# Yujia-Yan/Transkun

Hardware: AMD Instinct MI355X
Metric: semi-CRF logProb+backward steps/sec at T=1024, NBatch=352 (higher is better)
Workload: dtype f32; 1 GPU; NeuralSemiCRFInterval(score, noise).logProb(intervals) fwd+bwd through the public API (Python interval lists packed inside the timed region), T=1024, NBatch=352 per GPU, fp32, exact-hash randn-like scores resident in HBM; T=1024, NBatch=352, impl=0, parallelism=chains sharded, 1 rank(s) seen by the process group, no data-path collective

## Files before the change

transkun_amd/csrc/persist.hip:

```cpp
#include <atomic>
#include <stdlib.h>
#include "common.h"
#include "pathscore.h"

#ifndef SEMICRF_PANEL_PROBES
#define SEMICRF_PANEL_PROBES 0
#endif

#ifndef SEMICRF_PROBE_TASKS
#define SEMICRF_PROBE_TASKS 0
#endif
#ifndef SEMICRF_PROBE_HIST
#define SEMICRF_PROBE_HIST 0
#endif

#ifndef SEMICRF_CT_DBG
#define SEMICRF_CT_DBG -1
#endif

namespace semicrf {

constexpr int PB = 16;
#ifndef SEMICRF_RING
#define SEMICRF_RING 4
#endif
constexpr int RING = SEMICRF_RING;
#ifndef SEMICRF_NNEAR
#define SEMICRF_NNEAR 0
#endif
constexpr int NNEAR = SEMICRF_NNEAR;
#ifndef SEMICRF_BANDX
#define SEMICRF_BANDX 1
#endif
#ifndef SEMICRF_BANDX_MAXB
#define SEMICRF_BANDX_MAXB 192
#endif
#ifndef SEMICRF_BAND_LOAD_AUX
#define SEMICRF_BAND_LOAD_AUX 16
#endif
#ifndef SEMICRF_BANDX_WGSTRIDE
#define SEMICRF_BANDX_WGSTRIDE 3
#endif
#ifndef SEMICRF_BANDX_WAVES
#define SEMICRF_BANDX_WAVES 1
#endif
#ifndef SEMICRF_BANDX_K0
#define SEMICRF_BANDX_K0 8
#endif
constexpr int NBT = RING + NNEAR;
constexpr int FAR0 = RING + NNEAR;
constexpr int RS = 4;
constexpr int GS = RS;
constexpr int GP = 32;
#ifndef SEMICRF_TPT
#define SEMICRF_TPT 12
#endif
constexpr int TPT = SEMICRF_TPT;
#ifndef SEMICRF_LEADT
#define SEMICRF_LEADT 4
#endif
constexpr int LEADT = SEMICRF_LEADT;
__host__ __device__ inline int nfull_of(int q) { return q + 1 - LEADT >= 0 ? (q + 1 - LEADT) / TPT : 0; }
__host__ __device__ inline int nparts_of(int q) { return nfull_of(q) + 1; }
__host__ __device__ inline void part_tiles(int q, int part, int& m0, int& m1)
{
    m0 = part * TPT;
    m1 = part < nfull_of(q) ? m0 + TPT : q + 1;
}
#ifndef SEMICRF_NT
#define SEMICRF_NT 640
#endif
constexpr int NT = SEMICRF_NT;
constexpr int MAX_CHUNKS = 16;
constexpr float LOG2E = 1.4426950408889634f;
constexpr float LN2 = 0.6931471805599453f;
constexpr int SPIN_LIMIT = 1 << 20;
constexpr int SPIN_LIMIT_LDS = 1 << 24;
constexpr float RESC_LIFT = 96.0f, RESC_HI = 108.0f, RESC_EARLY = 56.0f;
constexpr unsigned CTRL_INIT = 0xffffffffu;
constexpr unsigned U_EMPTY = 0xffffffffu;

constexpr size_t CTRL_WORDS = 256;
constexpr int CTRL_EXIT = 64;
constexpr int CTRL_COPYQ = 192;
constexpr int CTRL_PATHQ = 160;
constexpr int CTRL_GEN = 96;

typedef unsigned long long u64;
typedef unsigned v4u __attribute__((ext_vector_type(4)));
typedef unsigned v4u_a4 __attribute__((ext_vector_type(4), aligned(4)));
template <int V>
struct IC { static constexpr int value = V; };

#define DBGF(P) (SEMICRF_CT_DBG >= 0 ? (unsigned)SEMICRF_CT_DBG : (P).dbg)
struct SweepParams {
    const float* score;
    const float* noise;
    int T, B, K;
    int c0, c1;
    int nSpine, nPanelGroups;
    int nTasks;
    int taskBase;
    int panelWaves;
    int hybridPanelWaves;
    int hybridStart;
    int zeroWaves;
    unsigned tag;
    int selfclean;
    unsigned expect_gen;
    unsigned dbg;
    unsigned* ctrl;
    u64* ts;
    unsigned* ug;
    unsigned* ug_other;
    int gradLazyShort;
    int bandWaves;
    u64* farg;
    float* u_out;
    float* last_out;
    int* code;
    const float* vfwd;
    const float* logZ;
    const float* gout;
    int gstride;
    float gscale;
    float* dScore;
    float* dNoise;
    const int* pathPairs;
    const int* pathOffsets;
    int pathK;
    int pathSpine;
    float* pathOut;
    u64* pathg;
    float noiseAdd;
    float* band;
    unsigned* bandFlags;
    int bandSpines;
    int bandGroups;
    int bandK0;
    int copyWaves;
    int cellNT;
    int gradNT;
    int nfarw;
};

__device__ __forceinline__ float fexp2(float x) { return __builtin_amdgcn_exp2f(x); }
__device__ __forceinline__ float flog2(float x) { return __builtin_amdgcn_logf(x); }

__device__ __forceinline__ u64 make_granule(unsigned tag, float v)
{
    return ((u64)tag << 32) | (u64)__float_as_uint(v);
}
__device__ __forceinline__ u64 make_granule_key(unsigned tag, float v, int key)
{
    return ((u64)(((tag & 0xffffu) << 16) | ((unsigned)key & 0xffffu)) << 32) | (u64)__float_as_uint(v);
}
__device__ __forceinline__ void store_granule(u64* p, u64 g)
{
    __hip_atomic_store(p, g, __ATOMIC_RELAXED, __HIP_MEMORY_SCOPE_AGENT);
}
__device__ __forceinline__ u64 load_granule(const u64* p)
{
    return __hip_atomic_load(p, __ATOMIC_RELAXED, __HIP_MEMORY_SCOPE_AGENT);
}

template <int DIR>
__device__ __forceinline__ int frame_of(int p, int T) { return DIR == 0 ? p : T - 1 - p; }

template <int DIR>
__device__ __forceinline__ size_t cell_index(int pi, int pj, int T)
{
    return DIR == 0 ? (size_t)pi * T + pj : (size_t)(T - 1 - pj) * T + (T - 1 - pi);
}
template <int DIR>
__device__ __forceinline__ int gap_of(int p, int T) { return DIR == 0 ? p - 1 : T - 1 - p; }

__device__ __forceinline__ void acc_push1(float& M, float& S, float t)
{
    const float d = t - M;
    const float e = fexp2(-fabsf(d));
    S = d > 0.0f ? fmaf(S, e, 1.0f) : S + e;
    M = fmaxf(M, t);
}
__device__ __forceinline__ void acc_merge(float& M, float& S, float M2, float S2)
{
    if (S2 == 0.0f) return;
    if (M2 > M) {
        S = S * fexp2(M - M2) + S2;
        M = M2;
    } else {
        S += S2 * fexp2(M2 - M);
    }
}
template <int DIR>
__device__ __forceinline__ void max_push_seq(float& best, int& key, float t, int k)
{
    const bool take = DIR == 0 ? t > best : t >= best;
    best = take ? t : best;
    key = take ? k : key;
}
__device__ __forceinline__ float softplus2(float x)
{
    const float x2 = x * LOG2E;
    return x > 20.0f ? x2 : flog2(1.0f + fexp2(x2));
}

__device__ unsigned g_dev_status = 0;
__shared__ int s_abort;

__device__ unsigned* g_host_abort = nullptr;

__device__ __forceinline__ void set_error(unsigned* ctrl, unsigned code)
{
    __hip_atomic_store(ctrl + 1, code, __ATOMIC_RELAXED, __HIP_MEMORY_SCOPE_AGENT);
    __hip_atomic_store(&g_dev_status, code, __ATOMIC_RELAXED, __HIP_MEMORY_SCOPE_AGENT);
    unsigned* const h = g_host_abort;
    if (h) __hip_atomic_store(h, code, __ATOMIC_RELAXED, __HIP_MEMORY_SCOPE_SYSTEM);
}

__device__ __forceinline__ bool spin_abort(unsigned* ctrl, int& spins, int limit, unsigned code)
{
    ++spins;
    if (spins > limit) { set_error(ctrl, code); s_abort = 1; return true; }
    if ((spins & 255) == 0 &&
        __hip_atomic_load(ctrl + 1, __ATOMIC_RELAXED, __HIP_MEMORY_SCOPE_AGENT) != CTRL_INIT) { s_abort = 1; return true; }
    return false;
}

#ifndef SEMICRF_NLOADER
#define SEMICRF_NLOADER 1
#endif
constexpr int NLOADER = SEMICRF_NLOADER;
#ifndef SEMICRF_NRBUF
#define SEMICRF_NRBUF 4
#endif
constexpr int NRBUF = SEMICRF_NRBUF;
constexpr int TILE_BYTES = PB * PB * RS * 4;
constexpr int NCONST = 3;
constexpr int LDS_TILES = 0;
constexpr int LDS_CONST = LDS_TILES + NRBUF * RING * TILE_BYTES;
constexpr int LDS_FAR = LDS_CONST + NRBUF * NCONST * 256;
constexpr int NFAR = 8;
constexpr int NPOS = 128;
static_assert(NFAR >= RING && NPOS >= RING * PB, "ring geometry");
constexpr int LDS_RING = LDS_FAR + NFAR * 64 * 16;
#ifndef SEMICRF_STAGGER
#define SEMICRF_STAGGER 32
#endif
#ifndef SEMICRF_GRAD_LAZY
#define SEMICRF_GRAD_LAZY 127
#endif
#ifndef SEMICRF_GRAD_HSTART
#define SEMICRF_GRAD_HSTART 12
#endif
#ifndef SEMICRF_LOADER_PACE
#define SEMICRF_LOADER_PACE 0
#endif
#ifndef SEMICRF_LOADER_AUX
#define SEMICRF_LOADER_AUX 0
#endif
#ifndef SEMICRF_SPH
#define SEMICRF_SPH 1
#endif
#ifndef SEMICRF_FAR_EARLY
#define SEMICRF_FAR_EARLY 0
#endif
#ifndef SEMICRF_FAR_PRIO
#define SEMICRF_FAR_PRIO 0
#endif
#ifndef SEMICRF_NFARW
#define SEMICRF_NFARW 2
#endif
constexpr int NFARW = SEMICRF_NFARW;
constexpr int NNSLOT = 8;
constexpr int NEAR_SLOT_BYTES = NNEAR * TILE_BYTES + 256;
constexpr int LDS_NEAR = LDS_RING + NPOS * RS * 8;
constexpr int LDS_CTL = LDS_NEAR + (NNEAR > 0 ? NNSLOT * NEAR_SLOT_BYTES : 0);
static_assert(NPOS >= (FAR0 + 1) * PB && NNSLOT >= FAR0 + 1 && NRBUF + RING + NNSLOT + NFARW <= 64 && NNSLOT % NFARW == 0, "near geometry");
constexpr int LDS_DUMMY = LDS_CTL + 256;
constexpr int LDS_SPINE_BYTES = LDS_DUMMY + (64 * 2 + PB * 8) * 4;

typedef __attribute__((address_space(3))) void lds_void_t;
typedef __attribute__((address_space(1))) const void gbl_void_t;

struct SpineBlk { float v[PB]; };

__device__ __forceinline__ int spine_row(int lane) { return lane & 15; }
__device__ __forceinline__ int spine_chain(int lane) { return lane >> 4; }

template <int N>
__device__ __forceinline__ void wait_vmcnt() { asm volatile("s_waitcnt vmcnt(%0)" ::"n"(N)); }

__device__ __forceinline__ int lds_flag_load(const int* p) { return __hip_atomic_load(p, __ATOMIC_RELAXED, __HIP_MEMORY_SCOPE_WORKGROUP); }
__device__ __forceinline__ void lds_flag_store(int* p, int v) { __hip_atomic_store(p, v, __ATOMIC_RELAXED, __HIP_MEMORY_SCOPE_WORKGROUP); }
__device__ __forceinline__ unsigned lds_addr(const void* p)
{
    return (unsigned)(uintptr_t)(__attribute__((address_space(3))) const void*)p;
}
__device__ __forceinline__ int lds_flag_load_asm(const int* p)
{
    int v;
    asm volatile("ds_read_b32 %0, %1\n\ts_waitcnt lgkmcnt(0)" : "=v"(v) : "v"(lds_addr(p)) : "memory");
    return v;
}
__device__ __forceinline__ void lds_flag_store_asm(int* p, int v)
{
    asm volatile("ds_write_b32 %0, %1" ::"v"(lds_addr(p)), "v"(v) : "memory");
}
__device__ __forceinline__ u64 lds_load64(const void* p)
{
    return __hip_atomic_load((const u64*)p, __ATOMIC_RELAXED, __HIP_MEMORY_SCOPE_WORKGROUP);
}
__device__ __forceinline__ void lds_store64(void* p, float value, int seq)
{
    __hip_atomic_store((u64*)p, ((u64)(unsigned)seq << 32) | (u64)__float_as_uint(value), __ATOMIC_RELAXED, __HIP_MEMORY_SCOPE_WORKGROUP);
}
typedef float f32x4_t __attribute__((ext_vector_type(4)));
__device__ __forceinline__ void lds_store128(void* p, float4 v)
{
    const f32x4_t w = {v.x, v.y, v.z, v.w};
    asm volatile("ds_write_b128 %0, %1" ::"v"(lds_addr(p)), "v"(w) : "memory");
}
__device__ __forceinline__ float4 lds_load128(const void* p)
{
    f32x4_t w;
    asm volatile("ds_read_b128 %0, %1\n\ts_waitcnt lgkmcnt(0)" : "=v"(w) : "v"(lds_addr(p)) : "memory");
    return make_float4(w.x, w.y, w.z, w.w);
}

template <int DIR, bool GRAD>
__device__ __forceinline__ void loader_role(const SweepParams& P, int sg, char* lds, int lid)
{
    const int T = P.T, B = P.B, K = P.K;
    unsigned* const ctrl = P.ctrl;
    const size_t Bs = (size_t)B;
    const float* const score = P.score;
    const float* const noise = P.noise;
    const float* const vfwd = P.vfwd;
    const int lane = threadIdx.x & 63;
    const int cbase = P.c0 + sg * GS;
    const size_t last4 = (size_t)T * T * Bs - 4;
    const int tu = lane >> 4, tr = lane & 15;
    const int cr = spine_row(lane), cch = spine_chain(lane);
    const int cc = cbase + cch < P.c1 ? cbase + cch : cbase;
    int* const ready = (int*)(lds + LDS_CTL);
    int* const cons = ready + NRBUF;
    int* const nready = cons + RING;
    const int* const fcons = nready + NNSLOT;
    constexpr int NL = RING * 4 + 2 + (GRAD ? 1 : 0) + NNEAR * 4 + ((GRAD && NNEAR > 0) ? 1 : 0);
    constexpr int LDEPTH = 3 * NL <= 63 ? 3 : 2;
    static_assert(2 * NL <= 63, "loader pipeline");

    const bool useband = SEMICRF_BANDX && P.band != nullptr;
    const float* const bandp = useband ? P.band + (size_t)(cbase / GS) * NBT * (TILE_BYTES / 4) + lane * 4 : nullptr;
    const size_t band_kr = (size_t)P.bandSpines * NBT * (TILE_BYTES / 4);
    typedef unsigned v16u __attribute__((ext_vector_type(16)));
    const int bKpad = K + 2;
    const unsigned* const bflags = useband ? P.bandFlags + (size_t)(cbase / GP) * bKpad * 8 : nullptr;
    const unsigned btag = P.tag;
    int ready_upto = -1;
    auto band_ready = [&](int kr) -> bool {
        const uintptr_t fa = (uintptr_t)(bflags + (size_t)kr * 8);
        const u64 fp = (u64)(unsigned)__builtin_amdgcn_readfirstlane((int)(unsigned)fa) |
                       ((u64)(unsigned)__builtin_amdgcn_readfirstlane((int)(unsigned)(fa >> 32)) << 32);
        v16u f;
        asm volatile("s_load_dwordx16 %0, %1, 0x0 glc\n\ts_waitcnt lgkmcnt(0)" : "=&s"(f) : "s"(fp) : "memory");
        const unsigned want0 = ((btag & 0xffffu) << 16) | (unsigned)kr, want1 = want0 + 1u;
        bool ok0 = true, ok1 = true;
#pragma unroll
        for (int i = 0; i < NBT; ++i) { ok0 = ok0 && f[i] == want0; ok1 = ok1 && f[8 + i] == want1; }
        if (ok0) ready_upto = ok1 ? kr + 1 : kr;
        return ok0;
    };
    auto issue = [&](int kr) {
        const int slot = kr % NRBUF;
        const int prow_t = kr * PB + tr < T ? kr * PB + tr : T - 1;
        const bool fromband = useband && kr >= P.bandK0;
        if (fromband) {
            const float* const bk = bandp + (size_t)kr * band_kr;
#pragma unroll
            for (int i = 0; i < RING; ++i)
#pragma unroll
                for (int q = 0; q < 4; ++q)
                    __builtin_amdgcn_global_load_lds((gbl_void_t*)(bk + i * (TILE_BYTES / 4) + q * 256),
                                                     (lds_void_t*)(lds + LDS_TILES + (slot * RING + i) * TILE_BYTES + q * 1024), 16, 0, SEMICRF_BAND_LOAD_AUX);
// ... 754 lines not shown
        const int c = c0 + g * GP + q8 * 4;
        const bool cvalid = c < c1;
        const int cl = cvalid ? c : c0;

        float aM[4][4], aS[4][4];
        int aK[4][4];
#pragma unroll
        for (int rr = 0; rr < 4; ++rr)
#pragma unroll
            for (int i = 0; i < 4; ++i) { aM[rr][i] = SEMICRF_NEG_INF; aS[rr][i] = 0.f; aK[rr][i] = 0x7fffffff; }

        float arow[4][4], gz[4];
        if (GRAD) {
            float lz[4];
#pragma unroll
            for (int i = 0; i < 4; ++i) {
                const bool ok = c + i < c1;
                lz[i] = ok ? logZp[c + i] : 0.f;
                gz[i] = ok ? goutp[(size_t)(c + i) * P.gstride] * P.gscale : 0.f;
            }
#pragma unroll
            for (int rr = 0; rr < 4; ++rr) {
                const int pi = pbase + rr;
#pragma unroll
                for (int i = 0; i < 4; ++i) {
                    const float vv = (c + i < c1 && pi < T) ? vfwd[(size_t)frame_of<DIR>(pi, T) * Bs + c + i] : 0.f;
                    arow[rr][i] = (vv - lz[i]) * LOG2E;
                }
            }
        }
        PanelGeom G;
        geom_of(tk, G);
        char* const stage0 = lds + wslot * (PNS * PSTAGE_BYTES);
        const unsigned rdbase = lds_addr(stage0) + (DIR == 0 ? (unsigned)lane * 16u
                                                             : (unsigned)((slot >> 1) * 1024 + (slot & 1) * 128 + q8 * 16));
        const unsigned grbase = lds_addr(stage0) + 8192u + (unsigned)lane * 16u;
        const bool probe_stream = SEMICRF_PANEL_PROBES && (dbg & 32u);
        const bool probe_nowait = SEMICRF_PANEL_PROBES && (dbg & 4u);
        const bool probe_nou = SEMICRF_PANEL_PROBES && (dbg & 64u);
        const int nst = GRAD ? 2 * (T - pbase < 4 ? T - pbase : 4) : 0;

        bool frontier = false;
#pragma unroll
        for (int i = 0; i < PNS; ++i)
            if (m0 + i < m1) {
                panel_fetch_cells<DIR>(score, G, stage0 + i * PSTAGE_BYTES, m0 + i, T, Bs, cell_nt);
                if (!probe_stream && !probe_nou) panel_fetch_gran<false>(ursrc, stage0 + i * PSTAGE_BYTES, G.gvoff, m0 + i, B);
                issued += 10;
                if (i == 0) mark0 = issued; else if (i == 1) mark1 = issued; else mark2 = issued;
            }

        for (int m = m0, s = 0; m < m1; ++m, s = (s + 1 == PNS ? 0 : s + 1)) {
            char* const stage = stage0 + s * PSTAGE_BYTES;
            const bool tprobe = SEMICRF_PANEL_PROBES && (dbg & 16u) && g == 0 && q4 == 0 && m == q && lane == 0 && k < 64 && T >= 1024;
            if (tprobe) P.ts[1536 + k] = __builtin_amdgcn_s_memrealtime();
            panel_wait_younger(issued - (s == 0 ? mark0 : (s == 1 ? mark1 : mark2)));
            if (tprobe) P.ts[1600 + k] = __builtin_amdgcn_s_memrealtime();
            int npoll = 0;
            if (tr && m == m0) tsp[1] = __builtin_amdgcn_s_memrealtime();
            if (SEMICRF_PROBE_HIST && (dbg & 1024u) && lane == 0) {
                u64* const hb = P.ts + (3 * T) / 2;
                const u64 now = __builtin_amdgcn_s_memrealtime();
                const u64 t0 = __hip_atomic_load(hb + 129 + (__builtin_amdgcn_s_getreg(6164) & 7), __ATOMIC_RELAXED, __HIP_MEMORY_SCOPE_AGENT);
                u64 b = now > t0 ? (now - t0) / 400 : 0;
                if (b > 63) b = 63;
                atomicAdd((unsigned long long*)(hb + 1 + 64 * hist_role + b), 1ull);
            }
            v4u xo[8];
            panel_read_cells<DIR>(rdbase + (unsigned)(s * PSTAGE_BYTES), xo);
            const bool refill = m + PNS < m1;
            if (probe_stream) {
#pragma unroll
                for (int e = 0; e < 8; ++e)
                    aS[0][0] += __uint_as_float(xo[e].x) + __uint_as_float(xo[e].y) + __uint_as_float(xo[e].z) + __uint_as_float(xo[e].w);
            } else {
                v4u g0, g1;
                panel_read_gran(grbase + (unsigned)(s * PSTAGE_BYTES), g0, g1);
                if (!probe_nowait) {
                    const bool v0 = c < c1, v1 = c + 1 < c1, v2 = c + 2 < c1, v3 = c + 3 < c1;
                    int spins = 0;
                    while (true) {
                        const bool ok = (g0.x != U_EMPTY || !v0) && (g0.y != U_EMPTY || !v1) && (g0.z != U_EMPTY || !v2) &&
                                        (g0.w != U_EMPTY || !v3) && (g1.x != U_EMPTY || !v0) && (g1.y != U_EMPTY || !v1) &&
                                        (g1.z != U_EMPTY || !v2) && (g1.w != U_EMPTY || !v3);
                        if (__all(ok)) break;
                        frontier = true;
                        if (m == q) __builtin_amdgcn_s_sleep(2);
                        else if (GRAD) {
                            if (P.gradLazyShort) __builtin_amdgcn_s_sleep(16);
                            else __builtin_amdgcn_s_sleep(SEMICRF_GRAD_LAZY);
                        }
                        else __builtin_amdgcn_s_sleep(16);
                        if (spin_abort(ctrl, spins, SPIN_LIMIT, 5)) break;
                        ++npoll;
                        if (m == q) panel_fetch_gran<true>(ursrc, stage, G.gvoff, m, B);
                        const unsigned pw = __builtin_amdgcn_raw_buffer_load_b32(ursrc, (unsigned)(cl * 4), (unsigned)((m * PB + PB - 1) * B * 4), 16);
                        if (!__all(pw != U_EMPTY || !cvalid)) continue;
                        if (m != q) panel_fetch_gran<true>(ursrc, stage, G.gvoff, m, B);
                        wait_vmcnt<0>();
                        panel_read_gran(grbase + (unsigned)(s * PSTAGE_BYTES), g0, g1);
                    }
                }
                if (frontier && m + 1 < m1) {
                    const int sn = s + 1 == PNS ? 0 : s + 1;
                    panel_fetch_gran<true>(ursrc, stage0 + sn * PSTAGE_BYTES, G.gvoff, m + 1, B);
                    issued += 2;
                    if (sn == 0) mark0 = issued; else if (sn == 1) mark1 = issued; else mark2 = issued;
                }
                if (SEMICRF_PANEL_PROBES && (dbg & 16u) && g == 0 && q4 == 0 && m == q && lane == 0) P.ts[192 + k] = __builtin_amdgcn_s_memrealtime();
                if (c >= c1) { g0.x = 0u; g1.x = 0u; }
                if (c + 1 >= c1) { g0.y = 0u; g1.y = 0u; }
                if (c + 2 >= c1) { g0.z = 0u; g1.z = 0u; }
                if (c + 3 >= c1) { g0.w = 0u; g1.w = 0u; }
                const float uv[2][4] = {{__uint_as_float(g0.x), __uint_as_float(g0.y), __uint_as_float(g0.z), __uint_as_float(g0.w)},
                                        {__uint_as_float(g1.x), __uint_as_float(g1.y), __uint_as_float(g1.z), __uint_as_float(g1.w)}};

                if (MODE == 0) {
                    typedef float v2f __attribute__((ext_vector_type(2)));
                    const v2f l2e = {LOG2E, LOG2E};
                    const v2f u2[2][2] = {{{uv[0][0], uv[0][1]}, {uv[0][2], uv[0][3]}}, {{uv[1][0], uv[1][1]}, {uv[1][2], uv[1][3]}}};
                    const auto gs = __builtin_amdgcn_make_buffer_rsrc((void*)(GRAD ? dScore + panel_tile_off<DIR>(G, m, T, Bs) : nullptr), 0,
                                                                      0x7fffffff, 0x00020000);
#pragma unroll
                    for (int rr = 0; rr < 4; ++rr) {
                        v2f e[2][2];
#pragma unroll
                        for (int h = 0; h < 2; ++h) {
                            const v4u xv = xo[rr * 2 + h];
                            const v2f x2[2] = {{__uint_as_float(xv.x), __uint_as_float(xv.y)}, {__uint_as_float(xv.z), __uint_as_float(xv.w)}};
#pragma unroll
                            for (int j = 0; j < 2; ++j) {
                                const v2f mj = {aM[rr][2 * j], aM[rr][2 * j + 1]};
                                e[h][j] = __builtin_elementwise_fma(x2[j], l2e, u2[h][j] - mj);
                            }
                        }
                        const float emax = fmaxf(fmaxf(fmaxf(e[0][0].x, e[0][0].y), fmaxf(e[0][1].x, e[0][1].y)),
                                                 fmaxf(fmaxf(e[1][0].x, e[1][0].y), fmaxf(e[1][1].x, e[1][1].y)));
                        if (__any(emax > RESC_HI)) {
#pragma unroll
                            for (int i = 0; i < 4; ++i) {
                                const float x0 = __uint_as_float(i == 0 ? xo[rr * 2].x : (i == 1 ? xo[rr * 2].y : (i == 2 ? xo[rr * 2].z : xo[rr * 2].w)));
                                const float x1 = __uint_as_float(i == 0 ? xo[rr * 2 + 1].x : (i == 1 ? xo[rr * 2 + 1].y : (i == 2 ? xo[rr * 2 + 1].z : xo[rr * 2 + 1].w)));
                                const float t0 = fmaf(x0, LOG2E, uv[0][i]), t1 = fmaf(x1, LOG2E, uv[1][i]);
                                acc_lift(aM[rr][i], aS[rr][i], fmaxf(t0, t1));
                                const float e0 = t0 - aM[rr][i], e1 = t1 - aM[rr][i];
                                if (i & 1) { e[0][i >> 1].y = e0; e[1][i >> 1].y = e1; } else { e[0][i >> 1].x = e0; e[1][i >> 1].x = e1; }
                            }
                        }
                        v2f mg[2][2];
#pragma unroll
                        for (int j = 0; j < 2; ++j) {
                            v2f sj = {aS[rr][2 * j], aS[rr][2 * j + 1]};
                            const v2f p0 = {fexp2(e[0][j].x), fexp2(e[0][j].y)};
                            const v2f p1 = {fexp2(e[1][j].x), fexp2(e[1][j].y)};
                            sj = (sj + p0) + p1;
                            aS[rr][2 * j] = sj.x; aS[rr][2 * j + 1] = sj.y;
                            if (GRAD) {
                                const v2f mj = {aM[rr][2 * j], aM[rr][2 * j + 1]};
                                const v2f aj = {arow[rr][2 * j], arow[rr][2 * j + 1]};
                                const v2f fa = mj + aj;
                                const v2f gzj = {gz[2 * j], gz[2 * j + 1]};
                                const v2f fx = {fexp2(fa.x), fexp2(fa.y)};
                                const v2f gF = gzj * fx;
                                mg[0][j] = gF * p0;
                                mg[1][j] = gF * p1;
                            }
                        }
                        if (GRAD) {
#pragma unroll
                            for (int h = 0; h < 2; ++h) {
                                if (cvalid && pbase + rr < T) {
                                    const unsigned so = panel_soff<DIR>(G, rr, h, T, Bs);
                                    v4u gv;
                                    gv.x = __float_as_uint(mg[h][0].x);
                                    gv.y = __float_as_uint(mg[h][0].y);
                                    gv.z = __float_as_uint(mg[h][1].x);
                                    gv.w = __float_as_uint(mg[h][1].y);
#ifdef SEMICRF_NO_PANEL_GSTORE
                                    asm volatile("" ::"v"(gv));
                                    continue;
#endif
                                    if (c + 3 < c1) {
                                        if (grad_nt) __builtin_amdgcn_raw_buffer_store_b128(gv, gs, G.voff, so, GRAD_AUX);
                                        else __builtin_amdgcn_raw_buffer_store_b128(gv, gs, G.voff, so, 0);
                                    }
                                    else {
                                        __builtin_amdgcn_raw_buffer_store_b32(gv.x, gs, G.voff, so, 0);
                                        if (c + 1 < c1) __builtin_amdgcn_raw_buffer_store_b32(gv.y, gs, G.voff + 4, so, 0);
                                        if (c + 2 < c1) __builtin_amdgcn_raw_buffer_store_b32(gv.z, gs, G.voff + 8, so, 0);
                                    }
                                }
                            }
                        }
                        __builtin_amdgcn_sched_barrier(0);
                    }
                    if (GRAD) issued += nst;
                } else {
#pragma unroll
                    for (int rr = 0; rr < 4; ++rr)
#pragma unroll
                        for (int h = 0; h < 2; ++h) {
                            const v4u xv = xo[rr * 2 + h];
                            const float xe[4] = {__uint_as_float(xv.x), __uint_as_float(xv.y), __uint_as_float(xv.z), __uint_as_float(xv.w)};
                            const int key = frame_of<DIR>(m * PB + slot + 8 * h, T);
#pragma unroll
                            for (int i = 0; i < 4; ++i) max_push_seq<DIR>(aM[rr][i], aK[rr][i], uv[h][i] + xe[i], key);
                        }
                }
            }
            if (tprobe) { P.ts[1664 + k] = __builtin_amdgcn_s_memrealtime(); P.ts[1792 + k] = (u64)npoll; }
            if (refill) {
                panel_fetch_cells<DIR>(score, G, stage, m + PNS, T, Bs, cell_nt);
                if (!probe_stream && !probe_nou) panel_fetch_gran<false>(ursrc, stage, G.gvoff, m + PNS, B);
                issued += 10;
                if (s == 0) mark0 = issued; else if (s == 1) mark1 = issued; else mark2 = issued;
            }
        }
        if (tr) { tsp[2] = __builtin_amdgcn_s_memrealtime(); tsp[4] = (u64)(m1 - m0) | ((u64)k << 8) | ((u64)(frontier ? 1 : 0) << 16) | ((u64)part << 20); }
        if (!(GRAD && MODE == 0)) wait_vmcnt<0>();
        (void)frontier;
        if (SEMICRF_PANEL_PROBES && (dbg & 16u) && g == 0 && q4 == 0 && m1 == q + 1 && lane == 0 && k < 64 && T >= 1024)
            P.ts[1728 + k] = __builtin_amdgcn_s_memrealtime();

        const bool b5 = (lane & 32) != 0, b4 = (lane & 16) != 0, b3 = (lane & 8) != 0;
        u64* fbase = farg + (size_t)part * T * Bs;
        const int pi = pbase + (b5 ? 2 : 0) + (b4 ? 1 : 0);
        {
            constexpr int RSTR = 65 * 8;
            char* const rb = stage0;
#pragma unroll
            for (int rr = 0; rr < 4; ++rr)
#pragma unroll
                for (int i = 0; i < 4; ++i)
                    *(float2*)(rb + (rr * 4 + i) * RSTR + lane * 8) =
                        make_float2(aM[rr][i], MODE == 0 ? aS[rr][i] : __int_as_float(aK[rr][i]));
            const int orow = (b5 ? 2 : 0) + (b4 ? 1 : 0);
#pragma unroll
            for (int e = 0; e < 2; ++e) {
                const int oi = (b3 ? 2 : 0) + e;
                const char* src = rb + (orow * 4 + oi) * RSTR + q8 * 8;
                float2 v[8];
#pragma unroll
                for (int j = 0; j < 8; ++j) v[j] = *(const float2*)(src + j * 64);
                const int cc = c + oi;
                u64 gr;
                if (MODE == 0) {
                    float mx = v[0].x;
#pragma unroll
                    for (int j = 1; j < 8; ++j) mx = fmaxf(mx, v[j].x);
                    float sum = 0.f;
#pragma unroll
                    for (int j = 0; j < 8; ++j) sum += v[j].y == 0.0f ? 0.0f : v[j].y * fexp2(v[j].x - mx);
                    gr = make_granule(tag, mx + flog2(sum));
                } else {
                    float bm = v[0].x;
                    int bk = __float_as_int(v[0].y);
#pragma unroll
                    for (int j = 1; j < 8; ++j) max_push(bm, bk, v[j].x, __float_as_int(v[j].y));
                    gr = make_granule_key(tag, bm, bk);
                }
                if (pi < T && cc < c1 && !(SEMICRF_PANEL_PROBES && (dbg & 32u))) store_granule(fbase + (size_t)pi * Bs + cc, gr);
            }
        }
        if (SEMICRF_PANEL_PROBES && (dbg & 16u) && g == 0 && m1 == q + 1 && lane == 0 && k < 64)
            P.ts[256 + 64 * q4 + k] = __builtin_amdgcn_s_memrealtime();
        if (tr) tsp[3] = __builtin_amdgcn_s_memrealtime();
        ++tn;
    }
}

__device__ __forceinline__ void zero_row(float* __restrict__ dScore, int e, int T, int B, int lane)
{
    const size_t n = (size_t)(T - 1 - e) * B;
    float* rowp = dScore + ((size_t)e * T + e + 1) * B;
    const size_t lead = (4 - (((uintptr_t)rowp >> 2) & 3)) & 3;
    const size_t head = lead < n ? lead : n;
    const size_t n4 = (n - head) / 4;
    typedef float f32x4 __attribute__((ext_vector_type(4)));
    f32x4* v = (f32x4*)(rowp + head);
    const f32x4 z = {0.f, 0.f, 0.f, 0.f};
    for (size_t i = lane; i < n4; i += 64) __builtin_nontemporal_store(z, v + i);
    if ((size_t)lane < head) rowp[lane] = 0.f;
    const size_t tail0 = head + n4 * 4;
    if (tail0 + lane < n) rowp[tail0 + lane] = 0.f;
}
__device__ __forceinline__ void zero_role(const SweepParams& P)
{
    const int T = P.T, B = P.B;
    float* const dScore = P.dScore;
    unsigned* const ctrl = P.ctrl;
    const int lane = threadIdx.x & 63;
    const int npairs = T / 2;
    while (true) {
        int p = 0;
        if (lane == 0) p = (int)(atomicAdd(ctrl + 3, 1u) + 1u);
        p = __builtin_amdgcn_readfirstlane(p);
        if (p >= npairs) break;
        const int e2 = T - 2 - p;
        if (p <= e2) zero_row(dScore, p, T, B, lane);
        if (p < e2) zero_row(dScore, e2, T, B, lane);
    }
}

constexpr int CTRL_BANDQ = 32;

template <int DIR>
__device__ __forceinline__ void band_role(const SweepParams& P)
{
    const int T = P.T, B = P.B, K = P.K, c0 = P.c0, c1 = P.c1;
    const size_t Bs = (size_t)B;
    unsigned* const ctrl = P.ctrl;
    const float* __restrict__ score = P.score;
    float* const dScore = P.dScore;
    const int lane = threadIdx.x & 63;
    const int q8 = lane & 7, pjsub = (lane >> 3) & 1, pisub = lane >> 4;
    const int nG = P.nPanelGroups;
    const int nTasks = K * FAR0 * nG * 4;
    const size_t last4 = (size_t)T * T * Bs - 4;
    const auto ursrc = __builtin_amdgcn_make_buffer_rsrc((void*)P.ug, 0, (int)((size_t)T * Bs * 4), 0x00020000);
    const bool grad_nt = __builtin_amdgcn_readfirstlane(P.gradNT) != 0;
    while (true) {
        int task = 0;
        if (lane == 0) task = (int)(atomicAdd(ctrl + CTRL_BANDQ, 1u) + 1u);
        task = __builtin_amdgcn_readfirstlane(task);
        if (task >= nTasks) break;
        const int q4 = task & 3, t2 = task >> 2;
        const int g = t2 % nG, t3 = t2 / nG;
        const int dk = t3 % FAR0, m = t3 / FAR0, k = m + dk;
        const int pbase = k * PB + q4 * 4;
        if (k >= K || pbase >= T) continue;
#if defined(SEMICRF_BAND_ABL) && SEMICRF_BAND_ABL == 2
        continue;
#endif
        const int pi = pbase + pisub;
        const bool rowok = pi < T;
        const int pic = rowok ? pi : T - 1;
        const int c = c0 + g * GP + q8 * 4;
        const int cl = c < c1 ? c : c0;
        const bool v0 = c < c1, v1 = c + 1 < c1, v2 = c + 2 < c1, v3 = c + 3 < c1;
        float gz[4], ar[4];
        {
            const int fr = frame_of<DIR>(pic, T);
#pragma unroll
            for (int i = 0; i < 4; ++i) {
                const bool ok = c + i < c1;
                const float lz = ok ? P.logZ[c + i] : 0.f;
                gz[i] = ok ? P.gout[(size_t)(c + i) * P.gstride] * P.gscale : 0.f;
                ar[i] = ok ? (P.vfwd[(size_t)fr * Bs + c + i] - lz) * LOG2E : 0.f;
            }
        }
        v4u x[8], uu[8];
        size_t off[8];
        unsigned uoff[8];
        bool use[8];
#pragma unroll
        for (int e = 0; e < 8; ++e) {
            const int pj = m * PB + 2 * e + pjsub;
            use[e] = rowok && pj < pi;
            const int pjc = pj < pic ? pj : (pic > 0 ? pic - 1 : 0);
            off[e] = cell_index<DIR>(pic, pjc, T) * Bs + cl;
            uoff[e] = (unsigned)(((size_t)pjc * Bs + cl) * 4);
            const v4u_a4 t = *(const v4u_a4*)(score + (off[e] < last4 ? off[e] : last4));
            x[e] = t;
            uu[e] = __builtin_amdgcn_raw_buffer_load_b128(ursrc, uoff[e], 0, 0);
        }
        {
            int spins = 0;
            while (true) {
                bool ok = true;
#pragma unroll
                for (int e = 0; e < 8; ++e)
                    ok = ok && (uu[e].x != U_EMPTY || !v0) && (uu[e].y != U_EMPTY || !v1) && (uu[e].z != U_EMPTY || !v2) && (uu[e].w != U_EMPTY || !v3);
                if (__all(ok)) break;
                __builtin_amdgcn_s_sleep(64);
                if (spin_abort(ctrl, spins, SPIN_LIMIT, 14)) break;
#pragma unroll
                for (int e = 0; e < 8; ++e) uu[e] = __builtin_amdgcn_raw_buffer_load_b128(ursrc, uoff[e], 0, 16);
            }
        }
#pragma unroll
        for (int e = 0; e < 8; ++e) {
            if (!use[e] || !v0) continue;
            v4u gv;
            gv.x = __float_as_uint(gz[0] * fexp2(fmaf(__uint_as_float(x[e].x), LOG2E, __uint_as_float(uu[e].x)) + ar[0]));
            gv.y = __float_as_uint(gz[1] * fexp2(fmaf(__uint_as_float(x[e].y), LOG2E, __uint_as_float(uu[e].y)) + ar[1]));
            gv.z = __float_as_uint(gz[2] * fexp2(fmaf(__uint_as_float(x[e].z), LOG2E, __uint_as_float(uu[e].z)) + ar[2]));
            gv.w = __float_as_uint(gz[3] * fexp2(fmaf(__uint_as_float(x[e].w), LOG2E, __uint_as_float(uu[e].w)) + ar[3]));
            float* const dst = dScore + off[e];
#if defined(SEMICRF_BAND_ABL) && SEMICRF_BAND_ABL == 1
            asm volatile("" ::"v"(gv));
            continue;
#endif
            if (v3) {
                const v4u_a4 ga = gv;
                if (grad_nt) __builtin_nontemporal_store(ga, (v4u_a4*)dst);
                else *(v4u_a4*)dst = ga;
            }
            else {
                dst[0] = __uint_as_float(gv.x);
                if (v1) dst[1] = __uint_as_float(gv.y);
                if (v2) dst[2] = __uint_as_float(gv.z);
            }
        }
    }
}

__device__ __forceinline__ void path_role(const SweepParams& P)
{
    const int nb = P.c1 - P.c0;
    while (true) {
        int i = 0;
        if ((threadIdx.x & 63) == 0) i = (int)(atomicAdd(P.ctrl + CTRL_PATHQ, 1u) + 1u);
        i = __builtin_amdgcn_readfirstlane(i);
        if (i >= nb) break;
        const int c = P.c0 + i;
        const double r = path_score_wave(P.score, P.noise, P.T, P.B, P.pathK, P.pathPairs, P.pathOffsets, c);
        __builtin_amdgcn_wave_barrier();
        store_granule(P.pathg + c, make_granule(P.tag, (float)r));
    }
}

__host__ __device__ __forceinline__ int wg_ticket(int nSpine, int grid, int b)
{
    constexpr int X = 8, SPG = GP / GS / SPH;
    const int ngroups = (nSpine + SPG - 1) / SPG;
    int S[X], W[X];
    bool fits = true;
#pragma unroll
    for (int x = 0; x < X; ++x) {
        W[x] = x < grid ? (grid - x + X - 1) / X : 0;
        int sx = 0;
        for (int g = x; g < ngroups; g += X) sx += nSpine - g * SPG < SPG ? nSpine - g * SPG : SPG;
        S[x] = sx;
        fits = fits && sx <= W[x];
    }
    if (!fits) return b;
    const int x = b % X, slot = b / X;
    int Sx = 0, Px = 0;
#pragma unroll
    for (int i = 0; i < X; ++i) if (i == x) { Sx = S[i]; Px = W[i] - S[i]; }
    (void)Px;
    if (slot < Sx) return (x + X * (slot / SPG)) * SPG + slot % SPG;
    const int ps = slot - Sx;
    int rank = 0;
#pragma unroll
    for (int i = 0; i < X; ++i) {
        const int pn = W[i] - S[i];
        rank += ps < pn ? ps : pn;
        if (i < x && pn > ps) ++rank;
    }
    return nSpine + rank;
}

template <int MODE, int DIR, bool GRAD>
__global__ __launch_bounds__(NT) void persist_sweep_kernel(SweepParams P)
{
    extern __shared__ __attribute__((aligned(16))) char s_dyn[];
    __shared__ int s_exit;
    if (threadIdx.x == 0) {
        const unsigned e1 = __hip_atomic_load(P.ctrl + 1, __ATOMIC_RELAXED, __HIP_MEMORY_SCOPE_AGENT);
        const unsigned gen = P.selfclean ? __hip_atomic_load(P.ctrl + CTRL_GEN, __ATOMIC_RELAXED, __HIP_MEMORY_SCOPE_AGENT) : P.expect_gen;
        s_abort = e1 != CTRL_INIT ? 1 : 0;
        if (gen != P.expect_gen) { set_error(P.ctrl, 13u); s_abort = 1; }
        s_exit = 0;
    }
    for (int h = 0; h < SPH; ++h)
        for (int i = threadIdx.x; i < (LDS_DUMMY - LDS_FAR) / 4; i += NT) ((int*)(s_dyn + h * LDS_HALF + LDS_FAR))[i] = 0;
    __syncthreads();
    const int nSpineWG = (P.nSpine + SPH - 1) / SPH;
    const int ticket = wg_ticket(nSpineWG, (int)gridDim.x, (int)blockIdx.x);
    const int wave = (int)(threadIdx.x >> 6);
    if (P.ug_other && wave == NT / 64 - 1) {
        const size_t n = (size_t)P.T * P.B, n4 = n / 4;
        const size_t per = (n4 + gridDim.x - 1) / gridDim.x, i0 = per * blockIdx.x, i1 = i0 + per < n4 ? i0 + per : n4;
        const v4u e = {U_EMPTY, U_EMPTY, U_EMPTY, U_EMPTY};
        for (size_t i = i0 + (threadIdx.x & 63); i < i1; i += 64) ((v4u*)P.ug_other)[i] = e;
        if (blockIdx.x == 0 && (threadIdx.x & 63) < (int)(n - n4 * 4)) P.ug_other[n4 * 4 + (threadIdx.x & 63)] = U_EMPTY;
    }
    const bool clk = SEMICRF_PANEL_PROBES && (DBGF(P) & 128u) && ticket == nSpineWG + 3 && threadIdx.x == 0;
    if (clk) { P.ts[600] = __builtin_readcyclecounter(); P.ts[601] = __builtin_amdgcn_s_memrealtime(); }
    if (SEMICRF_PROBE_HIST && (DBGF(P) & 1024u) && threadIdx.x == 0) {
        const unsigned long long now = (unsigned long long)__builtin_amdgcn_s_memrealtime();
        atomicMin((unsigned long long*)(P.ts + (3 * P.T) / 2), now);
        atomicMin((unsigned long long*)(P.ts + (3 * P.T) / 2 + 129 + (__builtin_amdgcn_s_getreg(6164) & 7)), now);
    }
    if (ticket < nSpineWG) {
        const int half = wave / HWAVES, hw = wave % HWAVES;
        const int sg = ticket * SPH + half;
        char* const lds_h = s_dyn + half * LDS_HALF;
        if (half >= SPH) {
            const int xw = wave - SPH * HWAVES;
            if (SPH == 1 && NFARW > 1 && wave >= NT / 64 - (NFARW - 1)) {
                if (ticket < P.nSpine && !(DBGF(P) & 9u)) far_role<MODE, DIR, GRAD>(P, ticket, s_dyn, 1 + wave - (NT / 64 - (NFARW - 1)));
            } else if (!(DBGF(P) & 2u) && xw < P.hybridPanelWaves) {
                {
                    const int* cons = (const int*)(s_dyn + LDS_CTL) + NRBUF;
                    int spins = 0;
                    while (lds_flag_load(cons + (P.hybridStart % RING)) < P.hybridStart + 1 && P.hybridStart < P.K &&
                           !(SEMICRF_PANEL_PROBES && (DBGF(P) & 8u))) {
                        __builtin_amdgcn_s_sleep(127);
                        if (spin_abort(P.ctrl, spins, SPIN_LIMIT_LDS, 10)) break;
                    }
                }
                panel_role<MODE, DIR, GRAD>(P, s_dyn + LDS_HYBRID_PANEL, xw, 1);
            } else if (MODE == 0 && DIR == 0 && !GRAD && P.pathPairs != nullptr && P.pathSpine && xw == P.hybridPanelWaves) {
                path_role(P);
            }
        } else if (sg >= P.nSpine) {
        } else if (hw < RING) {
            if (!(DBGF(P) & 8u)) {
                if (GRAD && P.bandWaves == 0) spine_role<MODE, DIR, GRAD, GRAD>(P, sg, hw, lds_h);
                else spine_role<MODE, DIR, GRAD, false>(P, sg, hw, lds_h);
            }
        } else if (hw < RING + NLOADER) {
            if (!(DBGF(P) & 8u)) loader_role<DIR, GRAD>(P, sg, lds_h, hw - RING);
        } else {
            if (!(DBGF(P) & 9u)) far_role<MODE, DIR, GRAD>(P, sg, lds_h, hw - (RING + NLOADER));
        }
    } else {
        if (!(DBGF(P) & 2u) && wave < P.panelWaves)
            panel_role<MODE, DIR, GRAD>(P, s_dyn, wave, 0, P.taskBase > 0 ? (ticket - nSpineWG) * P.panelWaves + wave : -1);
        else if (GRAD && wave - P.panelWaves >= 0 && wave - P.panelWaves < P.zeroWaves) zero_role(P);
        else if (GRAD && wave - P.panelWaves - P.zeroWaves >= 0 && wave - P.panelWaves - P.zeroWaves < P.bandWaves) band_role<DIR>(P);
        else if (SEMICRF_BANDX && wave >= NT / 64 - P.copyWaves && (ticket - nSpineWG) % SEMICRF_BANDX_WGSTRIDE == 0) copy_role<DIR>(P);
        else if (MODE == 0 && DIR == 0 && !GRAD && P.pathPairs != nullptr && wave == P.panelWaves) path_role(P);
    }
    if (clk) { P.ts[602] = __builtin_readcyclecounter(); P.ts[603] = __builtin_amdgcn_s_memrealtime(); }
    if (P.selfclean) {
        int left = 0;
        if ((threadIdx.x & 63) == 0) left = atomicAdd(&s_exit, 1) + 1;
        left = __builtin_amdgcn_readfirstlane(left);
        if (left == NT / 64) {
            unsigned before = 0;
            if ((threadIdx.x & 63) == 0) before = atomicAdd(P.ctrl + CTRL_EXIT, 1u) + 1u;
            before = (unsigned)__builtin_amdgcn_readfirstlane((int)before);
            if (before + 1u == gridDim.x &&
                __hip_atomic_load(P.ctrl + 1, __ATOMIC_RELAXED, __HIP_MEMORY_SCOPE_AGENT) == CTRL_INIT) {
                for (int i = threadIdx.x & 63; i < (int)CTRL_WORDS; i += 64)
                    __hip_atomic_store(P.ctrl + i, i == CTRL_GEN ? P.tag : CTRL_INIT, __ATOMIC_RELAXED, __HIP_MEMORY_SCOPE_AGENT);
            }
        }
    }
}

template <int DIR>
__device__ __forceinline__ void band_copy_load(const float* __restrict__ score, int T, int B, int kr, int g, int t, int q, int lane,
                                               v4u_a4 (&v)[8])
{
    const int q8 = lane & 7, cs = lane >> 3;
    const int cbase = (g * (GP / GS) + q8) * GS;
    const size_t Bs = (size_t)B;
    const size_t last4 = (size_t)T * T * Bs - 4;
    const int kc = kr - t > 0 ? kr - t : 0;
#pragma unroll
    for (int it = 0; it < 8; ++it) {
        const int ci = q * 64 + it * 8 + cs;
        const int col = ci >> 4, tr = ci & 15;
        const int prow_t = kr * PB + tr < T ? kr * PB + tr : T - 1;
        int pj = kc * PB + col;
        pj = pj < prow_t ? pj : (prow_t > 0 ? prow_t - 1 : 0);
        size_t off = cell_index<DIR>(prow_t, pj, T) * Bs + (cbase < B ? cbase : 0);
        off = off < last4 ? off : last4;
        v[it] = *(const v4u_a4*)(score + off);
    }
}
__device__ __forceinline__ void band_copy_store(float* __restrict__ band, int B, int bandSpines, int kr, int g, int t, int q, int lane,
                                                const v4u_a4 (&v)[8])
{
    const int q8 = lane & 7, cs = lane >> 3;
    const int sgG = g * (GP / GS) + q8;
    if (sgG * GS >= B) return;
    const int ti = t < RING ? RING - 1 - t : t;
    const auto rs = __builtin_amdgcn_make_buffer_rsrc((void*)band, 0, 0x7fffffff, 0x00020000);
    const unsigned voff = (unsigned)(((((size_t)kr * bandSpines + sgG) * NBT + ti) * (TILE_BYTES / 4) + (q * 64 + cs) * 4) * 4);
#pragma unroll
    for (int it = 0; it < 8; ++it) __builtin_amdgcn_raw_buffer_store_b128(v[it], rs, voff + it * 128, 0, 16);
}

template <int DIR>
__device__ __forceinline__ void copy_role(const SweepParams& P)
{
    const int K = P.K, nG = P.nPanelGroups, g0 = P.c0 / GP;
    const int nTasks = (K - P.bandK0) * NBT * nG;
    const int lane = threadIdx.x & 63;
    while (true) {
        int task = 0;
        if (lane == 0) task = (int)(atomicAdd(P.ctrl + CTRL_COPYQ, 1u) + 1u);
        task = __builtin_amdgcn_readfirstlane(task);
        if (task >= nTasks) break;
        const int g = task % nG, t = (task / nG) % NBT, kr = P.bandK0 + task / (nG * NBT);
        v4u_a4 va[8], vb[8];
        band_copy_load<DIR>(P.score, P.T, P.B, kr, g0 + g, t, 0, lane, va);
        band_copy_load<DIR>(P.score, P.T, P.B, kr, g0 + g, t, 1, lane, vb);
        band_copy_store(P.band, P.B, P.bandSpines, kr, g0 + g, t, 0, lane, va);
        band_copy_load<DIR>(P.score, P.T, P.B, kr, g0 + g, t, 2, lane, va);
        band_copy_store(P.band, P.B, P.bandSpines, kr, g0 + g, t, 1, lane, vb);
        band_copy_load<DIR>(P.score, P.T, P.B, kr, g0 + g, t, 3, lane, vb);
        band_copy_store(P.band, P.B, P.bandSpines, kr, g0 + g, t, 2, lane, va);
        band_copy_store(P.band, P.B, P.bandSpines, kr, g0 + g, t, 3, lane, vb);
        asm volatile("s_waitcnt vmcnt(0)" ::: "memory");
        __builtin_amdgcn_wave_barrier();
        __hip_atomic_store(P.bandFlags + ((size_t)(g0 + g) * (K + 2) + kr) * 8 + t, ((P.tag & 0xffffu) << 16) | (unsigned)kr, __ATOMIC_RELAXED,
                           __HIP_MEMORY_SCOPE_AGENT);
    }
}

static bool band_in_sweep(int T, int B)
{
    const int K = (T + PB - 1) / PB;
    return SEMICRF_BANDX && B <= SEMICRF_BANDX_MAXB && K > SEMICRF_BANDX_K0 + FAR0;
}
static size_t band_flag_bytes(int T, int B)
{
    if (!band_in_sweep(T, B)) return 0;
    return align_up((size_t)((T + PB - 1) / PB + 2) * ((B + GP - 1) / GP) * 8 * sizeof(unsigned));
}
static size_t band_copy_bytes(int T, int B)
{
    if (!band_in_sweep(T, B)) return 0;
    return align_up((size_t)((T + PB - 1) / PB) * ((B + GS - 1) / GS) * NBT * TILE_BYTES);
}

constexpr size_t CTRL_BYTES = MAX_CHUNKS * CTRL_WORDS * sizeof(unsigned);

#ifndef SEMICRF_NT_MIN_MB
#define SEMICRF_NT_MIN_MB 240
#endif
#ifndef SEMICRF_GRAD_NT_MIN_MB
#define SEMICRF_GRAD_NT_MIN_MB 0
#endif
#ifndef SEMICRF_NFARW2_MAXB
#define SEMICRF_NFARW2_MAXB 192
#endif
#ifndef SEMICRF_NFARW2_MINT
#define SEMICRF_NFARW2_MINT 1024
#endif
#ifndef SEMICRF_NT_MISALIGNED
#define SEMICRF_NT_MISALIGNED 0
#endif
static bool cell_policy_nt(int T, int nb, int min_mb)
{
    const double mb = 4.0 * nb * ((double)T * (T + 1) / 2) / 1e6;
    return mb >= (double)min_mb;
}

static int max_parts(int T)
{
    const int K = (T + PB - 1) / PB;
    return K > FAR0 ? nparts_of(K - 1 - FAR0) : 1;
}

__global__ __launch_bounds__(256) void zero_upper_kernel(float* __restrict__ dScore, int T, int B)
{
    const int e = blockIdx.y;
    const size_t n = (size_t)(T - 1 - e) * B;
    float* rowp = dScore + ((size_t)e * T + e + 1) * B;
    const size_t lead = (4 - (((uintptr_t)rowp >> 2) & 3)) & 3;
    const size_t head = lead < n ? lead : n;
    const size_t n4 = (n - head) / 4;
    float4* v = (float4*)(rowp + head);
    for (size_t i = (size_t)blockIdx.x * 256 + threadIdx.x; i < n4; i += (size_t)gridDim.x * 256)
        v[i] = make_float4(0.f, 0.f, 0.f, 0.f);
    if (blockIdx.x == 0) {
        if (threadIdx.x < head) rowp[threadIdx.x] = 0.f;
        const size_t tail0 = head + n4 * 4;
        if (tail0 + threadIdx.x < n) rowp[tail0 + threadIdx.x] = 0.f;
    }
}

__global__ __launch_bounds__(256) void fill_ff_kernel(v4u* __restrict__ p, size_t n16)
{
    const v4u e = {0xffffffffu, 0xffffffffu, 0xffffffffu, 0xffffffffu};
    for (size_t i = (size_t)blockIdx.x * 256 + threadIdx.x; i < n16; i += (size_t)gridDim.x * 256) p[i] = e;
}

void launch_zero_upper(float* X, int T, int B, hipStream_t stream)
{
    if (T < 2) return;
    int gx = (int)(((size_t)T * B / 4 + 255) / 256);
    if (gx > 8) gx = 8;
    if (gx < 1) gx = 1;
    hipLaunchKernelGGL(zero_upper_kernel, dim3(gx, T - 1), dim3(256), 0, stream, X, T, B);
}

constexpr int MAX_DEVICES = 64;
static int current_device()
{
    int dev = 0;
    if (hipGetDevice(&dev) != hipSuccess || dev < 0 || dev >= MAX_DEVICES) dev = 0;
    return dev;
}
static int device_cus()
{
    static std::atomic<int> ncu[MAX_DEVICES];
    const int dev = current_device();
    int n = ncu[dev].load();
    if (n == 0) {
        int v = 0;
        n = 256;
// ... 234 lines not shown
```

Measured before the change: 1822 steps/s.

## Shard band task queue per XCD and use buffer stores for gradient tiles

Splits the single global band-role atomic work counter into one counter per XCD, read from a hardware register. Panel groups are interleaved across the queues so each XCD mostly drains its own queue and then steals from the others. This targets contention on one cross-die atomic and aims to keep each panel's writes local to one XCD. It also switches the full-width gradient stores to raw buffer stores relative to a per-task base, which adds work to compute the base and offsets.

After: 1749 steps/s. 4.0% lower.

```diff
diff --git a/transkun_amd/csrc/persist.hip b/transkun_amd/csrc/persist.hip
--- a/transkun_amd/csrc/persist.hip
+++ b/transkun_amd/csrc/persist.hip
@@ -80,7 +80,7 @@
 constexpr unsigned CTRL_INIT = 0xffffffffu;
 constexpr unsigned U_EMPTY = 0xffffffffu;
 
-constexpr size_t CTRL_WORDS = 256;
+constexpr size_t CTRL_WORDS = 512;
 constexpr int CTRL_EXIT = 64;
 constexpr int CTRL_COPYQ = 192;
 constexpr int CTRL_PATHQ = 160;
@@ -1441,7 +1441,13 @@
     }
 }
 
-constexpr int CTRL_BANDQ = 32;
+#ifndef SEMICRF_BANDQ_XCDS
+#define SEMICRF_BANDQ_XCDS 8
+#endif
+constexpr int NBQ = SEMICRF_BANDQ_XCDS;
+constexpr int CTRL_BANDQ = 256;
+static_assert(NBQ >= 1 && NBQ <= 8 && (NBQ & (NBQ - 1)) == 0, "band queues: 1, 2, 4 or 8");
+static_assert(CTRL_BANDQ + 32 * NBQ <= (int)CTRL_WORDS, "the band queue heads lie inside the control words");
 
 template <int DIR>
 __device__ __forceinline__ void band_role(const SweepParams& P)
@@ -1454,17 +1460,24 @@
     const int lane = threadIdx.x & 63;
     const int q8 = lane & 7, pjsub = (lane >> 3) & 1, pisub = lane >> 4;
     const int nG = P.nPanelGroups;
-    const int nTasks = K * FAR0 * nG * 4;
     const size_t last4 = (size_t)T * T * Bs - 4;
     const auto ursrc = __builtin_amdgcn_make_buffer_rsrc((void*)P.ug, 0, (int)((size_t)T * Bs * 4), 0x00020000);
     const bool grad_nt = __builtin_amdgcn_readfirstlane(P.gradNT) != 0;
+    const int xcd = (int)(__builtin_amdgcn_s_getreg(6164) & (unsigned)(NBQ - 1));
+    int qx = xcd, done = 0;
     while (true) {
+        const int nGq = qx < nG ? (nG - qx + NBQ - 1) / NBQ : 0;
+        const int nTasks = K * FAR0 * nGq * 4;
         int task = 0;
-        if (lane == 0) task = (int)(atomicAdd(ctrl + CTRL_BANDQ, 1u) + 1u);
+        if (lane == 0) task = (int)(atomicAdd(ctrl + CTRL_BANDQ + 32 * qx, 1u) + 1u);
         task = __builtin_amdgcn_readfirstlane(task);
-        if (task >= nTasks) break;
+        if (task >= nTasks) {
+            if (++done == NBQ) break;
+            qx = (qx + 1) & (NBQ - 1);
+            continue;
+        }
         const int q4 = task & 3, t2 = task >> 2;
-        const int g = t2 % nG, t3 = t2 / nG;
+        const int g = qx + NBQ * (t2 % nGq), t3 = t2 / nGq;
         const int dk = t3 % FAR0, m = t3 / FAR0, k = m + dk;
         const int pbase = k * PB + q4 * 4;
         if (k >= K || pbase >= T) continue;
@@ -1477,6 +1490,9 @@
         const int c = c0 + g * GP + q8 * 4;
         const int cl = c < c1 ? c : c0;
         const bool v0 = c < c1, v1 = c + 1 < c1, v2 = c + 2 < c1, v3 = c + 3 < c1;
+        const int pimax = pbase + 3 < T ? pbase + 3 : T - 1, pjmax = m * PB + PB - 1 < T - 1 ? m * PB + PB - 1 : T - 1;
+        const size_t tbase = (DIR == 0 ? cell_index<DIR>(pbase, m * PB, T) : cell_index<DIR>(pimax, pjmax, T)) * Bs;
+        const auto gsrc = __builtin_amdgcn_make_buffer_rsrc((void*)(dScore + tbase), 0, 0x7fffffff, 0x00020000);
         float gz[4], ar[4];
         {
             const int fr = frame_of<DIR>(pic, T);
@@ -1531,9 +1547,9 @@
             continue;
 #endif
             if (v3) {
-                const v4u_a4 ga = gv;
-                if (grad_nt) __builtin_nontemporal_store(ga, (v4u_a4*)dst);
-                else *(v4u_a4*)dst = ga;
+                const unsigned gvoff = (unsigned)((off[e] - tbase) * 4);
+                if (grad_nt) __builtin_amdgcn_raw_buffer_store_b128(gv, gsrc, gvoff, 0, GRAD_AUX);
+                else __builtin_amdgcn_raw_buffer_store_b128(gv, gsrc, gvoff, 0, 0);
             }
             else {
                 dst[0] = __uint_as_float(gv.x);
```
